# CityU-AIM-Group/SimT

Hardware: AMD Instinct MI355X
Metric: training images/sec at 768x768, DeepLabv2-R101+SimT (higher is better)
Workload: dtype bf16; 1 GPU; DeepLabv2-ResNet101 + SimT(C=19,K=3) full training iteration, batch=4/GPU, 768x768, bf16, 1xMI355X; global_batch=4, inputs=resident in HBM (see h2d_inclusive of a --full run for the PCIe-inclusive rate)

## Files before the change

### simt_amd/csrc/bn_pool.hip

```cpp
#include "common.h"

template <int NJ>
__device__ __forceinline__ void part_colsum8(const float* part, int nblk, int C, int c0, double* out , double (*red)[8][NJ]) {
  const int cl = threadIdx.x & 7, r = threadIdx.x >> 3;
  const int c = c0 + cl;
  double s[NJ];
#pragma unroll
  for (int j = 0; j < NJ; ++j) s[j] = 0.0;
  if (c < C) {
    int b = r;
    for (; b + 96 < nblk; b += 128) {
      float v[4][NJ];
#pragma unroll
      for (int u = 0; u < 4; ++u)
#pragma unroll
        for (int j = 0; j < NJ; ++j) v[u][j] = part[((long)(b + 32 * u) * NJ + j) * C + c];
#pragma unroll
      for (int u = 0; u < 4; ++u)
#pragma unroll
        for (int j = 0; j < NJ; ++j) s[j] += (double)v[u][j];
    }
    for (; b < nblk; b += 32)
#pragma unroll
      for (int j = 0; j < NJ; ++j) s[j] += (double)part[((long)b * NJ + j) * C + c];
// ... 471 lines not shown
    int b = (int)(t / Hp);
    float sc[8], sh[8], best[8];
    int bi[8];
    load8(scale + c, sc);
    load8(shift + c, sh);
#pragma unroll
    for (int e = 0; e < 8; ++e) { best[e] = -INFINITY; bi[e] = 0; }
    bool first = true;
    for (int r = 0; r < 3; ++r) {
      int iy = py * 2 - 1 + r;
      if (iy < 0 || iy >= H) continue;
      for (int s = 0; s < 3; ++s) {
        int ix = px * 2 - 1 + s;
        if (ix < 0 || ix >= W) continue;
        float v[8];
        load8(y + (((long)b * H + iy) * W + ix) * C + c, v);
#pragma unroll
        for (int e = 0; e < 8; ++e) {
          float a = v[e] * sc[e] + sh[e];
          a = a > 0.f ? a : 0.f;
          if (first || a > best[e] || a != a) { best[e] = a; bi[e] = r * 3 + s; }
        }
        first = false;
      }
    }
    store8(p + i * 8, best);
    unsigned long long packed = 0;
#pragma unroll
    for (int e = 0; e < 8; ++e) packed |= (unsigned long long)(bi[e] & 0xff) << (8 * e);
    *(unsigned long long*)(idx + i * 8) = packed;
  }
}

template <typename T>
__global__ void maxpool_bwd_kernel(const T* dp, const unsigned char* idx, T* da, int B, int H, int W, int C, int Hp,
                                   int Wp, long nvec) {
  const int vpr = C >> 3;
  for (long i = (long)blockIdx.x * blockDim.x + threadIdx.x; i < nvec; i += (long)gridDim.x * blockDim.x) {
    int c = (int)(i % vpr) << 3;
    long m = i / vpr;
    int ix = (int)(m % W);
    long t = m / W;
    int iy = (int)(t % H);
    int b = (int)(t / H);
    float acc[8];
#pragma unroll
    for (int e = 0; e < 8; ++e) acc[e] = 0.f;
    int py0 = iy >> 1, px0 = ix >> 1;
    for (int py = py0; py <= ((iy + 1) >> 1); ++py) {
      if (py >= Hp) continue;
      int r = iy - (py * 2 - 1);
      if (r < 0 || r > 2) continue;
      for (int px = px0; px <= ((ix + 1) >> 1); ++px) {
        if (px >= Wp) continue;
        int s = ix - (px * 2 - 1);
        if (s < 0 || s > 2) continue;
        long o = (((long)b * Hp + py) * Wp + px) * C + c;
        unsigned long long packed = *(const unsigned long long*)(idx + o);
        float g[8];
        load8(dp + o, g);
        int want = r * 3 + s;
#pragma unroll
        for (int e = 0; e < 8; ++e)
          if ((int)((packed >> (8 * e)) & 0xff) == want) acc[e] += g[e];
      }
    }
    store8(da + i * 8, acc);
  }
}

extern "C" int simt_bn_relu_maxpool(const void* y, const float* scale, const float* shift, void* p, unsigned char* idx,
                                    int B, int H, int W, int C, int Hp, int Wp, int dtype, simt_stream_t stream) {
  SIMT_CHECK(y && scale && shift && p && idx && C % 8 == 0);
  long nvec = (long)B * Hp * Wp * (C / 8);
  if (dtype == SIMT_BF16)
    hipLaunchKernelGGL(bn_relu_maxpool_kernel<bf16_t>, dim3(ew_grid(nvec)), dim3(256), 0, (hipStream_t)stream,
                       (const bf16_t*)y, scale, shift, (bf16_t*)p, idx, B, H, W, C, Hp, Wp, nvec);
  else
    hipLaunchKernelGGL(bn_relu_maxpool_kernel<float>, dim3(ew_grid(nvec)), dim3(256), 0, (hipStream_t)stream,
                       (const float*)y, scale, shift, (float*)p, idx, B, H, W, C, Hp, Wp, nvec);
  SIMT_LAUNCH_CHECK();
  return SIMT_OK;
}

extern "C" int simt_maxpool_bwd(const void* dp, const unsigned char* idx, void* da, int B, int H, int W, int C, int Hp,
                                int Wp, int dtype, simt_stream_t stream) {
  SIMT_CHECK(dp && idx && da && C % 8 == 0);
  long nvec = (long)B * H * W * (C / 8);
  if (dtype == SIMT_BF16)
    hipLaunchKernelGGL(maxpool_bwd_kernel<bf16_t>, dim3(ew_grid(nvec)), dim3(256), 0, (hipStream_t)stream,
                       (const bf16_t*)dp, idx, (bf16_t*)da, B, H, W, C, Hp, Wp, nvec);
  else
    hipLaunchKernelGGL(maxpool_bwd_kernel<float>, dim3(ew_grid(nvec)), dim3(256), 0, (hipStream_t)stream, (const float*)dp,
                       idx, (float*)da, B, H, W, C, Hp, Wp, nvec);
  SIMT_LAUNCH_CHECK();
  return SIMT_OK;
}

__device__ __forceinline__ long long frag_offset(long long row, long long kcol, int nt16) {
  const long long kt = kcol >> 6, s = (kcol >> 5) & 1, kq = (kcol >> 3) & 3, e = kcol & 7;
  const long long lane = (row & 15) | (kq << 4);
  return ((((kt * nt16 + (row >> 4)) * 2 + s) * 64 + lane) << 3) + e;
}
template <typename T>
__global__ void pack_weight_kernel(const float* w, T* dst, int Cout, int Cin, int RS, int row_off, int tap_off, long ldk,
                                   int Ck, int mode, const float* cscale, long total) {
  for (long i = (long)blockIdx.x * blockDim.x + threadIdx.x; i < total; i += (long)gridDim.x * blockDim.x) {
    int t = (int)(i % RS);
    long r = i / RS;
    int ci = (int)(r % Cin);
    int co = (int)(r / Cin);
    float v = w[i];
    if (cscale) v *= cscale[co];
    const int lm = mode & 0xff, nt16 = mode >> 8;
    const long row = lm == 0 ? (long)(row_off + co) : lm == 1 ? (long)ci : (long)(tap_off + t) * Ck + row_off + co;
    const long kcol = lm == 0 ? (long)(tap_off + t) * Cin + ci : lm == 1 ? (long)(tap_off + t) * Ck + row_off + co : (long)ci;
    const long o = nt16 ? (long)frag_offset(row, kcol, nt16) : row * ldk + kcol;
    Elem<T>::st(dst + o, v);
  }
}

extern "C" int simt_pack_weight(const float* w, void* dst, int Cout, int Cin, int RS, int row_off, int tap_off, long ldk,
                                int Ck, int mode, const float* cscale, int dtype, simt_stream_t stream) {
  SIMT_CHECK(w && dst && Cout > 0 && Cin > 0 && RS > 0);
  long total = (long)Cout * Cin * RS;
  if (dtype == SIMT_BF16)
    hipLaunchKernelGGL(pack_weight_kernel<bf16_t>, dim3(ew_grid(total)), dim3(256), 0, (hipStream_t)stream, w, (bf16_t*)dst,
// ... 312 lines not shown
```

### simt_amd/csrc/common.h

```cpp
#pragma once
#include <hip/hip_runtime.h>
#include <stdint.h>
#include "../../include/simt_hip.h"

typedef unsigned short bf16_t;
typedef __attribute__((ext_vector_type(8))) short bf16x8;
typedef __attribute__((ext_vector_type(4))) short bf16x4;
typedef __attribute__((ext_vector_type(4))) __bf16 bf4v;
typedef __attribute__((ext_vector_type(4))) float f32x4;
typedef __attribute__((ext_vector_type(4))) unsigned int u32x4;

#define GPTR(p) ((const __attribute__((address_space(1))) void*)(p))
#define LPTR(p) ((__attribute__((address_space(3))) void*)(p))

__device__ __forceinline__ float bf2f(bf16_t v) { return __uint_as_float(((uint32_t)v) << 16); }
__device__ __forceinline__ bf16_t f2bf(float f) {
  __bf16 b = (__bf16)f;
  return __builtin_bit_cast(bf16_t, b);
}

__device__ __forceinline__ uint32_t pack_bf16x2(float a, float b) {
  typedef __attribute__((ext_vector_type(2))) float f32x2_t;
  typedef __attribute__((ext_vector_type(2))) __bf16 bf16x2_t;
  const f32x2_t v = {a, b};
// ... 37 lines not shown
}
#ifndef SIMT_NT_STORES
#define SIMT_NT_STORES 0
#endif
static __device__ __forceinline__ void st_out16(void* p, const uint4& v) {
  typedef unsigned simt_u32x4 __attribute__((ext_vector_type(4)));
  const simt_u32x4 w = {v.x, v.y, v.z, v.w};
#if SIMT_NT_STORES
  __builtin_nontemporal_store(w, (simt_u32x4*)p);
#else
  *(simt_u32x4*)p = w;
#endif
}
static __device__ __forceinline__ void st_out8(bf16_t* p, const float* v) {
  uint4 r;
  r.x = pack_bf16x2(v[0], v[1]); r.y = pack_bf16x2(v[2], v[3]); r.z = pack_bf16x2(v[4], v[5]); r.w = pack_bf16x2(v[6], v[7]);
  st_out16(p, r);
}
static __device__ __forceinline__ void st_out8(float* p, const float* v) {
  st_out16(p, make_uint4(__float_as_uint(v[0]), __float_as_uint(v[1]), __float_as_uint(v[2]), __float_as_uint(v[3])));
  st_out16(p + 4, make_uint4(__float_as_uint(v[4]), __float_as_uint(v[5]), __float_as_uint(v[6]), __float_as_uint(v[7])));
}

static __device__ __forceinline__ void store8(float* p, const float* v) { st_out8(p, v); }
static __device__ __forceinline__ void store8(bf16_t* p, const float* v) { st_out8(p, v); }
static __device__ __forceinline__ void st_out16f(float* p, const f32x4& v) {
#if SIMT_NT_STORES
  __builtin_nontemporal_store(v, (f32x4*)p);
#else
  *(f32x4*)p = v;
#endif
}

__device__ __forceinline__ int xcd_remap(int bid, int nwg) {
  int q = nwg >> 3, r = nwg & 7, xcd = bid & 7;
  int base = xcd < r ? xcd * (q + 1) : r * (q + 1) + (xcd - r) * q;
  return base + (bid >> 3);
}

__device__ __forceinline__ float wave_sum(float v) {
#pragma unroll
  for (int o = 32; o > 0; o >>= 1) v += __shfl_xor(v, o, 64);
  return v;
}
__device__ __forceinline__ double wave_sum_d(double v) {
#pragma unroll
  for (int o = 32; o > 0; o >>= 1) v += __shfl_xor(v, o, 64);
  return v;
}

__device__ __forceinline__ void fast_divmod(int m, int d, float rcp, int& q, int& r) {
  q = (int)((float)m * rcp);
  r = m - q * d;
  if (r < 0) { q--; r += d; }
  if (r >= d) { q++; r -= d; }
}

#define SIMT_MAX_DEVICES 16
struct SimtLdsAttrCache { size_t set[SIMT_MAX_DEVICES]; };
static inline bool simt_lds_attr_needed(SimtLdsAttrCache* c, size_t lds) {
  int dev = 0;
  if (hipGetDevice(&dev) != hipSuccess || dev < 0 || dev >= SIMT_MAX_DEVICES) return true;
  if (lds <= c->set[dev]) return false;
  c->set[dev] = lds;
  return true;
}
// ... 20 lines not shown
```

### simt_amd/csrc/head_expand.hip

```cpp
#include "common.h"

struct TapArgs {
  const void* src;
  const float* bias;
  void* dst;
  int B, H, W, Q, QP, lds, ldd, ntaps;
  long M;
  short dy[SIMT_MAX_TAPS], dx[SIMT_MAX_TAPS];
};

__global__ __launch_bounds__(256) void tap_gather_sum_kernel(TapArgs a) {
  const int nq = a.QP >> 2;
  const long total = a.M * nq;
  const float* P = (const float*)a.src;
  float* y = (float*)a.dst;
  for (long idx = (long)blockIdx.x * blockDim.x + threadIdx.x; idx < total; idx += (long)gridDim.x * blockDim.x) {
    const int q = (int)(idx % nq);
    const long m = idx / nq;
    const int ox = (int)(m % a.W);
    const long t2 = m / a.W;
    const int oy = (int)(t2 % a.H);
    float4 acc = make_float4(0.f, 0.f, 0.f, 0.f);
    if (a.bias) {
      const int c = q * 4;
      acc.x = c + 0 < a.Q ? a.bias[c + 0] : 0.f;
      acc.y = c + 1 < a.Q ? a.bias[c + 1] : 0.f;
      acc.z = c + 2 < a.Q ? a.bias[c + 2] : 0.f;
      acc.w = c + 3 < a.Q ? a.bias[c + 3] : 0.f;
    }
    for (int t = 0; t < a.ntaps; ++t) {
      const int iy = oy + a.dy[t], ix = ox + a.dx[t];
      if (iy < 0 || iy >= a.H || ix < 0 || ix >= a.W) continue;
      const float4 v = *(const float4*)(P + (m + (long)a.dy[t] * a.W + a.dx[t]) * a.lds + t * a.QP + q * 4);
      acc.x += v.x; acc.y += v.y; acc.z += v.z; acc.w += v.w;
    }
    *(float4*)(y + m * a.ldd + q * 4) = acc;
  }
}

__global__ __launch_bounds__(256) void tap_scatter_kernel(TapArgs a) {
  const int ng = a.QP >> 3;
  const long total = a.M * a.ntaps * ng;
  const bf16_t* d = (const bf16_t*)a.src;
  bf16_t* G = (bf16_t*)a.dst;
  for (long idx = (long)blockIdx.x * blockDim.x + threadIdx.x; idx < total; idx += (long)gridDim.x * blockDim.x) {
    const int g = (int)(idx % ng);
    long r = idx / ng;
    const int t = (int)(r % a.ntaps);
    const long m = r / a.ntaps;
    const int ox = (int)(m % a.W);
    const int oy = (int)((m / a.W) % a.H);
    const int iy = oy - a.dy[t], ix = ox - a.dx[t];
    uint4 v = make_uint4(0u, 0u, 0u, 0u);
    if (iy >= 0 && iy < a.H && ix >= 0 && ix < a.W)
      v = *(const uint4*)(d + (m - ((long)a.dy[t] * a.W + a.dx[t])) * a.lds + g * 8);
    st_out16(G + m * a.ldd + t * a.QP + g * 8, v);
  }
}

static int tap_grid(long total) {
  long g = (total + 255) / 256;
  if (g > 256 * 16) g = 256 * 16;
  return (int)(g < 1 ? 1 : g);
}

extern "C" int simt_tap_gather_sum(const simt_tap_desc* d, simt_stream_t stream) {
  SIMT_CHECK(d && d->src && d->dst && d->ntaps >= 1 && d->ntaps <= SIMT_MAX_TAPS);
  SIMT_CHECK(d->QP % 4 == 0 && d->lds % 4 == 0 && d->ldd % 4 == 0 && d->QP <= d->ldd && d->ntaps * d->QP <= d->lds);
  TapArgs a;
  a.src = d->src; a.bias = d->bias; a.dst = d->dst; a.B = d->B; a.H = d->H; a.W = d->W; a.Q = d->Q; a.QP = d->QP;
  a.lds = d->lds; a.ldd = d->ldd; a.ntaps = d->ntaps; a.M = (long)d->B * d->H * d->W;
  for (int i = 0; i < SIMT_MAX_TAPS; ++i) { a.dy[i] = d->dy[i]; a.dx[i] = d->dx[i]; }
  hipLaunchKernelGGL(tap_gather_sum_kernel, dim3(tap_grid(a.M * (a.QP / 4))), dim3(256), 0, (hipStream_t)stream, a);
  SIMT_LAUNCH_CHECK();
  return SIMT_OK;
}

extern "C" int simt_tap_scatter(const simt_tap_desc* d, simt_stream_t stream) {
  SIMT_CHECK(d && d->src && d->dst && d->ntaps >= 1 && d->ntaps <= SIMT_MAX_TAPS);
  SIMT_CHECK(d->QP % 8 == 0 && d->lds % 8 == 0 && d->ldd % 8 == 0 && d->QP <= d->lds && d->ntaps * d->QP <= d->ldd);
  TapArgs a;
  a.src = d->src; a.bias = nullptr; a.dst = d->dst; a.B = d->B; a.H = d->H; a.W = d->W; a.Q = d->Q; a.QP = d->QP;
  a.lds = d->lds; a.ldd = d->ldd; a.ntaps = d->ntaps; a.M = (long)d->B * d->H * d->W;
  for (int i = 0; i < SIMT_MAX_TAPS; ++i) { a.dy[i] = d->dy[i]; a.dx[i] = d->dx[i]; }
  hipLaunchKernelGGL(tap_scatter_kernel, dim3(tap_grid(a.M * a.ntaps * (a.QP / 8))), dim3(256), 0, (hipStream_t)stream, a);
  SIMT_LAUNCH_CHECK();
  return SIMT_OK;
}
```

### simt_amd/csrc/head_loss.hip

```cpp
#include "common.h"
#include <math.h>

#define QMAX 40
#ifndef SIMT_HEAD_ABL
#define SIMT_HEAD_ABL 0
#endif
#define NSCAL 13
#define XR_MAX 287

struct HeadGeom {
  int B, h, w, H, W, C, Q, ldp, ldf;
  float sy, sx;
  int half;
  int fix_logits;
  int single;
};

__device__ __forceinline__ float src_coord(int half, float scale, int d) {
  return half ? fmaxf(((float)d + 0.5f) * scale - 0.5f, 0.f) : scale * (float)d;
}
__device__ __forceinline__ void dst_range(int l, int out, float scale, int& lo, int& hi) {
  if (scale > 0.f) {
    const float r = 1.f / scale;
    lo = (int)floorf(((float)l - 1.f) * r) - 2;
    hi = (int)ceilf(((float)l + 2.f) * r) + 2;
  } else { lo = 0; hi = out - 1; }
  lo = max(lo, 0); hi = min(hi, out - 1);
}

struct Taps {
  int o00, o01, o10, o11;
  float wy0, wy1, wx0, wx1;
};

__device__ __forceinline__ Taps make_taps(const HeadGeom& g, int b, int y, int x) {
  Taps t;
  float fy = src_coord(g.half, g.sy, y), fx = src_coord(g.half, g.sx, x);
  int iy0 = (int)fy, ix0 = (int)fx;
  if (iy0 > g.h - 1) iy0 = g.h - 1;
  if (ix0 > g.w - 1) ix0 = g.w - 1;
// ... 102 lines not shown
      m2 = fmaxf(m2, v[j]);
      if (j >= C && v[j] > best) { best = v[j]; y = j; }
    }
  float s2 = exp_le0(0.f - m2);
#pragma unroll
  for (int j = 0; j < QM; ++j)
    if (j < Q && j != arg) s2 += exp_le0(v[j] - m2);
  e.yopen = y; e.m2 = m2; e.sum2 = s2; e.lse2 = m2 + logf(s2);
}

__device__ __forceinline__ unsigned int f32_ord(float f) {
  unsigned int u = __float_as_uint(f);
  return (u & 0x80000000u) ? ~u : (u | 0x80000000u);
}
__device__ __forceinline__ float f32_unord(unsigned int o) {
  unsigned int u = (o & 0x80000000u) ? (o & 0x7fffffffu) : ~o;
  return __uint_as_float(u);
}

__global__ void softmax_rows_kernel(const float* in, int ldi, float* out, int ldo, long M, int C) {
  long m = (long)blockIdx.x * blockDim.x + threadIdx.x;
  if (m >= M) return;
  const float* p = in + m * ldi;
  float mx = p[0];
  for (int c = 1; c < C; ++c) mx = fmaxf(mx, p[c]);
  float s = 0.f;
  for (int c = 0; c < C; ++c) s += expf(p[c] - mx);
  float inv = 1.0f / s;
  float* o = out + m * ldo;
  for (int c = 0; c < C; ++c) o[c] = expf(p[c] - mx) * inv;
  for (int c = C; c < ldo; ++c) o[c] = 0.f;
}

extern "C" int simt_softmax_rows(const float* in, int ldi, float* out, int ldo, long M, int C, simt_stream_t stream) {
  SIMT_CHECK(in && out && C <= ldi && C <= ldo);
  hipLaunchKernelGGL(softmax_rows_kernel, dim3((unsigned)((M + 255) / 256)), dim3(256), 0, (hipStream_t)stream, in, ldi,
                     out, ldo, M, C);
  SIMT_LAUNCH_CHECK();
  return SIMT_OK;
}

struct HeadArgs {
  HeadGeom g;
  const float* pred1;
  const float* pred2;
  const float* fixp;
  const long long* label;
  const float* T1;
  const float* T2;
  float th_high, th_low, lambda_seg, lambda_place;
  float* part;
  unsigned long long* keys;
  float* hout;
  float* g1;
  int QP;
  int rows;
  float gscale;
  int mode;
  unsigned char* conf_out;
  unsigned char* label_ws;
};

__device__ __forceinline__ float wave_sum_dpp63(float v) {
  int x = __float_as_int(v);
#define DPP_ADD(ctrl, rmask)                                                                                  \
  x = __float_as_int(__int_as_float(x) + __int_as_float(__builtin_amdgcn_update_dpp(0, x, ctrl, rmask, 0xf, true)))
  DPP_ADD(0xB1, 0xf);
  DPP_ADD(0x4E, 0xf);
  DPP_ADD(0x141, 0xf);
  DPP_ADD(0x140, 0xf);
// ... 215 lines not shown
              long pp = grp * 256 + wave * 64 + (__ffsll((long long)b1) - 1);
              unsigned long long key = ((unsigned long long)f32_ord(m1) << 32) | (unsigned long long)(0xFFFFFFFFu - (unsigned int)pp);
              atomicMax(&sKey[j], key);
            }
          }
          if (__ballot(live && v2[j] >= best2)) {
            const float a2 = live ? v2[j] : -INFINITY;
            float m2 = wave_max_f(a2);
            unsigned long long b2 = __ballot(live && a2 == m2);
            if (lane == 0 && b2) {
              long pp = grp * 256 + wave * 64 + (__ffsll((long long)b2) - 1);
              unsigned long long key = ((unsigned long long)f32_ord(m2) << 32) | (unsigned long long)(0xFFFFFFFFu - (unsigned int)pp);
              atomicMax(&sKey[QMAX + j], key);
            }
          }
        }
    }
  }

#pragma unroll
  for (int i = 0; i < NSCAL; ++i) {
    float s = wave_sum(acc[i]);
    if (lane == 0) sRed[wave * NSCAL + i] = s;
  }
  __syncthreads();
  float* part = a.part + (long)lbid * (NSCAL + 2 * QC);
  if (tid < NSCAL) part[tid] = sRed[tid] + sRed[NSCAL + tid] + sRed[2 * NSCAL + tid] + sRed[3 * NSCAL + tid];
  for (int i = tid; i < 2 * QC; i += 256)
    part[NSCAL + i] = sdT[i] + sdT[2 * QC + i] + sdT[4 * QC + i] + sdT[6 * QC + i];
  if (tid < 2 * QMAX && sKey[tid]) atomicMax(&a.keys[tid], sKey[tid]);
  if (tid < 2 && sEx[tid]) atomicOr(&a.keys[2 * QMAX + tid], sEx[tid]);
}

__global__ __launch_bounds__(256) void head_reduce_kernel(const float* part, int nblk, int stride, int ncols, double* sums) {
  __shared__ double red[32][8];
  const int cl = threadIdx.x & 7, r = threadIdx.x >> 3;
  const int c = blockIdx.x * 8 + cl;
  double s = 0.0;
  if (c < ncols) {
    int b = r;
    for (; b + 96 < nblk; b += 128) {
      float v[4];
#pragma unroll
      for (int u = 0; u < 4; ++u) v[u] = part[(long)(b + 32 * u) * stride + c];
#pragma unroll
      for (int u = 0; u < 4; ++u) s += (double)v[u];
    }
    for (; b < nblk; b += 32) s += (double)part[(long)b * stride + c];
  }
  red[r][cl] = s;
  __syncthreads();
  if (r == 0 && c < ncols) {
    double t = 0.0;
#pragma unroll
    for (int q = 0; q < 32; ++q) t += red[q][cl];
    sums[c] = t;
  }
}

__device__ __forceinline__ double* head_sums(float* hout, int Q, int C) {
  return (double*)(hout + ((16 + 4 * Q * C + 4 * QMAX + 1) & ~1));
}

__global__ __launch_bounds__(256) void head_finalize_kernel(HeadArgs a, int nblk) {
  const HeadGeom g = a.g;
  const int Q = g.Q, C = g.C, QC = Q * C;
  const int tid = threadIdx.x;
  const double* sc = head_sums(a.hout, Q, C);
  float* o = a.hout;
  const double Np = sc[8], Nk1 = sc[9], Nk2 = sc[10], Ny = sc[11];
  if (tid == 0) {
    o[0] = (float)(sc[0] / Np); o[1] = (float)(sc[1] / Np);
    float k1 = (float)(sc[2] / Nk1), k2 = (float)(sc[3] / Nk2), u1 = (float)(sc[4] / Nk1), u2 = (float)(sc[5] / Nk2);
    o[2] = k1 + a.lambda_place * u1; o[3] = k2 + a.lambda_place * u2;
    o[4] = (float)(sc[6] / Ny); o[5] = (float)(sc[7] / Ny);
    o[6] = (float)Np; o[7] = (float)Nk1; o[8] = (float)Nk2; o[9] = (float)Ny;
    o[10] = k1; o[11] = k2; o[12] = u1; o[13] = u2;
    o[14] = o[1] + a.lambda_seg * o[0];
    o[15] = (float)sc[12];
  }
  float* dTy = o + 16 + 2 * QC + 4 * QMAX;
  for (int i = tid; i < 2 * QC; i += 256) dTy[i] = (float)(-sc[NSCAL + i] / Ny);
  float* ex = o + 16 + 2 * QC;
  float* ai = ex + 2 * QMAX;
  const unsigned long long e1 = a.keys[2 * QMAX], e2 = a.keys[2 * QMAX + 1];
  if (tid < 2 * QMAX) {
    int hd = tid / QMAX, j = tid % QMAX;
    ex[tid] = (j < Q && (((hd ? e2 : e1) >> j) & 1ull)) ? 1.f : 0.f;
    unsigned long long key = a.keys[tid];
    int pidx = (j < Q) ? (int)(0xFFFFFFFFu - (unsigned int)(key & 0xFFFFFFFFull)) : 0;
    ai[tid] = __int_as_float(pidx);
  }
  for (int i = tid; i < 2 * QC; i += 256) {
    if (a.mode != 0) { o[16 + i] = 0.f; continue; }
    int hd = i / QC, r = i % QC, j = r / C, c = r % C;
    unsigned long long key = a.keys[hd * QMAX + j];
    long p = (long)(0xFFFFFFFFu - (unsigned int)(key & 0xFFFFFFFFull));
    int x = (int)(p % g.W);
    long t = p / g.W;
    int y = (int)(t % g.H);
    int b = (int)(t / g.H);
    if (b >= g.B) { b = 0; y = 0; x = 0; }
    Taps tp = make_taps(g, b, y, x);
    const float* f = a.fixp;
    const float vc = lerp4(tp, f[(long)tp.o00 * g.ldf + c], f[(long)tp.o01 * g.ldf + c], f[(long)tp.o10 * g.ldf + c],
                           f[(long)tp.o11 * g.ldf + c]);
    if (!g.fix_logits) { o[16 + i] = vc; continue; }
    float mx = -INFINITY;
    for (int cc = 0; cc < C; ++cc)
      mx = fmaxf(mx, lerp4(tp, f[(long)tp.o00 * g.ldf + cc], f[(long)tp.o01 * g.ldf + cc], f[(long)tp.o10 * g.ldf + cc],
                           f[(long)tp.o11 * g.ldf + cc]));
    float sum = 0.f;
    for (int cc = 0; cc < C; ++cc)
      sum += expf(lerp4(tp, f[(long)tp.o00 * g.ldf + cc], f[(long)tp.o01 * g.ldf + cc], f[(long)tp.o10 * g.ldf + cc],
                        f[(long)tp.o11 * g.ldf + cc]) - mx);
    o[16 + i] = expf(vc - mx) / sum;
  }
}

template <int NB>
__device__ __forceinline__ float run_sum(const float* G, int GP, const float* sL1, int lo, int hi, int mode, float s) {
  if (SIMT_HEAD_ABL & 16) return s;
  float wv[NB * 4], gv[NB * 4];
#pragma unroll
  for (int u = 0; u < NB * 4; ++u) {
    const int pp = max(min(lo + u, hi - 1), 0);
    const float l1 = sL1[pp];
    const float w = mode == 0 ? l1 : mode == 2 ? (1.f - l1) + l1 : 1.f - l1;
    wv[u] = lo + u < hi ? w : 0.f;
    gv[u] = G[pp * GP];
  }
#pragma unroll
  for (int u = 0; u < NB * 4; ++u)
    if (wv[u] != 0.f) s += wv[u] * gv[u];
  return s;
}

#define P2_NACC 18
template <int QM, int QT, int CT, bool... ONE_>
__global__ __launch_bounds__(256, 2) void head_pass2_kernel(HeadArgs a) {
  constexpr bool ONE = (false || ... || ONE_);
  static_assert(!ONE || QT == 0, "the one-head warm-up flavour takes its channel counts at run time (rows = 1)");
  const HeadGeom g = a.g;
  const int Q = QT ? QT : g.Q, C = CT ? CT : g.C, QC = Q * C, QP = a.QP;
  constexpr int CM = CT ? (CT + 3) / 4 * 4 : QM;
  const int GP = Q + 1;
  extern __shared__ __attribute__((aligned(16))) char smem[];
  float* sT = (float*)smem;
  float* sG = sT + 2 * QC;
  float* sAcc = sG + 2 * 256 * GP;
// ... 216 lines not shown
    const float l1 = fy - (float)i0, l0 = 1.f - l1;
    float wk[3];
#pragma unroll
    for (int k = 0; k < 3; ++k) wk[k] = (i0 == iy_first + k ? l0 : 0.f) + (i1 == iy_first + k ? l1 : 0.f);
#pragma unroll
    for (int i = 0; i < NACC; ++i) {
      const int idx = tid + 256 * i;
      if (idx < 2 * g.w * Q) {
        const float sv = sAcc[idx];
#pragma unroll
        for (int k = 0; k < 3; ++k) gacc[k][i] += wk[k] * sv;
      }
    }
    __syncthreads();
  }
  }
  if (GROUPED && R > 1) {
    const int NG = g.H / R, gy = y0 / R;
#pragma unroll
    for (int i = 0; i < NACC; ++i) {
      const int idx = tid + 256 * i;
      if (idx < 2 * g.w * Q) {
        const int hd = idx / (g.w * Q);
        const int r = idx - hd * g.w * Q;
        const int xl = r / Q, j = r - xl * Q;
#pragma unroll
        for (int k = 0; k < 3; ++k)
          a.g1[(((((long)hd * g.B + b) * NG + gy) * 3 + k) * g.w + xl) * QP + j] = gacc[k][i];
      }
    }
  }
}

template <typename T>
__global__ void head_yreduce_kernel(const float* g1, float* d32_1, float* d32_2, T* dT_1, T* dT_2, HeadGeom g, int QP,
                                    int ldo32, int ldoT, long total, int R) {
  long idx = (long)blockIdx.x * blockDim.x + threadIdx.x;
  if (idx >= total) return;
  int j = (int)(idx % QP);
  long t = idx / QP;
  int xl = (int)(t % g.w); t /= g.w;
  int yl = (int)(t % g.h); t /= g.h;
  int b = (int)(t % g.B);
  int hd = (int)(t / g.B);
  if (g.single && hd == 0) return;
  int lo, hi;
  dst_range(yl, g.H, g.sy, lo, hi);
  float s = 0.f;
  if (R > 1) {
    const int NG = g.H / R;
    if (j < g.Q)
      for (int gy = lo / R; gy <= hi / R; ++gy) {
        const int k = yl - min((int)src_coord(g.half, g.sy, gy * R), g.h - 1);
        if (k >= 0 && k < 3) s += g1[(((((long)hd * g.B + b) * NG + gy) * 3 + k) * g.w + xl) * QP + j];
      }
  } else
  for (int yy = lo; yy <= hi; ++yy) {
    float fy = src_coord(g.half, g.sy, yy);
    int i0 = (int)fy;
    if (i0 > g.h - 1) i0 = g.h - 1;
    int i1 = i0 + (i0 < g.h - 1 ? 1 : 0);
    float l1 = fy - (float)i0, l0 = 1.f - l1;
    float wgt = (i0 == yl ? l0 : 0.f) + (i1 == yl ? l1 : 0.f);
    if (wgt != 0.f) s += wgt * g1[((((long)hd * g.B + b) * g.H + yy) * g.w + xl) * QP + j];
  }
  long m = ((long)b * g.h + yl) * g.w + xl;
  float* d32 = hd ? d32_2 : d32_1;
  T* dT = hd ? dT_2 : dT_1;
  if (d32 && j < ldo32) d32[m * ldo32 + j] = s;
  if (dT && j < ldoT) Elem<T>::st(dT + m * ldoT + j, s);
}

static size_t pass1_lds(int Q, int C) {
  size_t QC = (size_t)Q * C;
  return (2 * QC + 8 * QC) * 4 + 8 + (2 * QMAX + 2) * 8 + 4 * NSCAL * 4 + 16;
}
static size_t pass2_lds(int Q, int C, int w) {
  size_t QC = (size_t)Q * C;
  return (2 * QC + 2 * 256 * (size_t)(Q + 1) + 2 * (size_t)w * Q + 512 + XR_MAX + 1) * 4;
}

static int head_rows_per_block(const simt_head_desc* d, float sy) {
  const bool fixed_counts = d->C == 19 && (d->Q == 22 || d->Q == 25);
  if (!fixed_counts || 2l * d->w * d->Q > 256l * P2_NACC) return 1;
  for (int R = 8; R >= 3; --R)
    if (d->H % R == 0 && (float)(R - 1) * sy <= 0.95f && (long)d->B * d->H / R >= 512) return R;
  return 1;
// ... 9 lines not shown
  a.g.B = d->B; a.g.h = d->h; a.g.w = d->w; a.g.H = d->H; a.g.W = d->W; a.g.C = d->C; a.g.Q = d->Q;
  a.g.ldp = d->ldp; a.g.ldf = d->ldf;
  a.g.half = d->up_half_pixel ? 1 : 0; a.g.fix_logits = d->fix_logits ? 1 : 0; a.g.single = d->single ? 1 : 0;
  if (a.g.half) {
    a.g.sy = (float)d->h / (float)d->H;
    a.g.sx = (float)d->w / (float)d->W;
  } else {
    a.g.sy = d->H > 1 ? (float)(d->h - 1) / (float)(d->H - 1) : 0.f;
    a.g.sx = d->W > 1 ? (float)(d->w - 1) / (float)(d->W - 1) : 0.f;
  }
  a.pred1 = d->single ? d->pred2 : d->pred1; a.pred2 = d->pred2; a.fixp = d->fixp; a.label = (const long long*)d->label;
  a.T1 = d->single ? d->T2 : d->T1; a.T2 = d->T2;
  a.th_high = d->th_high; a.th_low = d->th_low; a.lambda_seg = d->lambda_seg; a.lambda_place = d->lambda_place;
  a.part = d->part; a.keys = (unsigned long long*)d->keys; a.hout = d->hout; a.g1 = d->g1; a.QP = d->QP;
  a.gscale = d->gscale;
  a.rows = (d->single && d->mode == 1) ? 1 : head_rows_per_block(d, a.g.sy);
  a.mode = d->mode;
  a.conf_out = d->conf_out;
  a.label_ws = d->label_ws;
  SIMT_CHECK(d->mode == 0 || d->mode == 1);
  return SIMT_OK;
}

extern "C" int simt_head_nblk(int B, int H, int W) {
  long P = (long)B * H * W;
  long n = (P + 255) / 256;
  if (n > 512) n = 512;
  return (int)n;
}
extern "C" int simt_head_part_floats(int Q, int C) { return NSCAL + 2 * Q * C; }
extern "C" int simt_head_hout_floats(int Q, int C) {
  return ((16 + 4 * Q * C + 4 * QMAX + 1) & ~1) + 2 * (NSCAL + 2 * Q * C);
}
extern "C" int simt_head_keys_count(void) { return 2 * QMAX + 2; }

extern "C" int simt_head_loss(const simt_head_desc* d, simt_stream_t stream) {
  HeadArgs a;
  int rc = fill_args(d, a);
  if (rc) return rc;
  hipStream_t st = (hipStream_t)stream;
  const int nblk = simt_head_nblk(d->B, d->H, d->W);
  (void)hipMemsetAsync(d->keys, 0, (2 * QMAX + 2) * sizeof(unsigned long long), st);
  size_t lds1 = pass1_lds(d->Q, d->C);
  SIMT_CHECK(lds1 <= 160 * 1024);
  static SimtLdsAttrCache lds1_cache;
  if (simt_lds_attr_needed(&lds1_cache, lds1)) {
#define P1ATTR(...) (void)hipFuncSetAttribute((const void*)head_pass1_kernel<__VA_ARGS__>, hipFuncAttributeMaxDynamicSharedMemorySize, (int)lds1)
    P1ATTR(24, 22, 19); P1ATTR(28, 25, 19); P1ATTR(24, 0, 0); P1ATTR(QMAX, 0, 0); P1ATTR(24, 0, 0, true); P1ATTR(QMAX, 0, 0, true);
#undef P1ATTR
  }
#define P1(...) hipLaunchKernelGGL((head_pass1_kernel<__VA_ARGS__>), dim3(nblk), dim3(256), lds1, st, a)
  const bool one = d->single && d->mode == 1;
  if (one && d->Q <= 24) P1(24, 0, 0, true);
  else if (one) P1(QMAX, 0, 0, true);
  else if (d->Q == 22 && d->C == 19) P1(24, 22, 19);
  else if (d->Q == 25 && d->C == 19) P1(28, 25, 19);
  else if (d->Q <= 24) P1(24, 0, 0);
  else P1(QMAX, 0, 0);
#undef P1
  SIMT_LAUNCH_CHECK();
  {
    const int ncols = NSCAL + 2 * d->Q * d->C;
    double* sums = (double*)(d->hout + ((16 + 4 * d->Q * d->C + 4 * QMAX + 1) & ~1));
    hipLaunchKernelGGL(head_reduce_kernel, dim3((ncols + 7) / 8), dim3(256), 0, st, d->part, nblk, ncols, ncols, sums);
    SIMT_LAUNCH_CHECK();
  }
  hipLaunchKernelGGL(head_finalize_kernel, dim3(1), dim3(256), 0, st, a, nblk);
  SIMT_LAUNCH_CHECK();
  return SIMT_OK;
}

extern "C" int simt_head_grad(const simt_head_desc* d, simt_stream_t stream) {
  HeadArgs a;
  int rc = fill_args(d, a);
  if (rc) return rc;
  SIMT_CHECK(d->g1 && d->QP >= d->Q);
  hipStream_t st = (hipStream_t)stream;
  size_t lds2 = pass2_lds(d->Q, d->C, d->w);
  SIMT_CHECK(lds2 <= 160 * 1024);
  static SimtLdsAttrCache lds2_cache;
  if (simt_lds_attr_needed(&lds2_cache, lds2)) {
#define P2ATTR(...) (void)hipFuncSetAttribute((const void*)head_pass2_kernel<__VA_ARGS__>, hipFuncAttributeMaxDynamicSharedMemorySize, (int)lds2)
    P2ATTR(24, 22, 19); P2ATTR(28, 25, 19); P2ATTR(24, 0, 0); P2ATTR(QMAX, 0, 0); P2ATTR(24, 0, 0, true); P2ATTR(QMAX, 0, 0, true);
#undef P2ATTR
  }
#define P2(...) hipLaunchKernelGGL((head_pass2_kernel<__VA_ARGS__>), dim3(d->B * d->H / a.rows), dim3(256), lds2, st, a)
  const bool one = d->single && d->mode == 1;
  if (one && d->Q <= 24) P2(24, 0, 0, true);
  else if (one) P2(QMAX, 0, 0, true);
  else if (d->Q == 22 && d->C == 19) P2(24, 22, 19);
  else if (d->Q == 25 && d->C == 19) P2(28, 25, 19);
  else if (d->Q <= 24) P2(24, 0, 0);
  else P2(QMAX, 0, 0);
#undef P2
  SIMT_LAUNCH_CHECK();
  long total = 2l * d->B * d->h * d->w * d->QP;
  unsigned grid = (unsigned)((total + 255) / 256);
  if (d->grad_dtype == SIMT_BF16)
    hipLaunchKernelGGL(head_yreduce_kernel<bf16_t>, dim3(grid), dim3(256), 0, st, d->g1, d->dpred1_f32, d->dpred2_f32,
                       (bf16_t*)d->dpred1_t, (bf16_t*)d->dpred2_t, a.g, d->QP, d->ld_f32, d->ld_t, total, a.rows);
  else
    hipLaunchKernelGGL(head_yreduce_kernel<float>, dim3(grid), dim3(256), 0, st, d->g1, d->dpred1_f32, d->dpred2_f32,
                       (float*)d->dpred1_t, (float*)d->dpred2_t, a.g, d->QP, d->ld_f32, d->ld_t, total, a.rows);
  SIMT_LAUNCH_CHECK();
  return SIMT_OK;
}
```

Baseline: 173.2 images/s.

## Cheapen index math, batch tap loads, fuse head reduce/finalize, vectorize softmax

Adds 32-bit index division when element counts fit, applied to the maxpool backward, tap gather/scatter and yreduce kernels. The 18-tap gather is fully unrolled so all loads are issued before accumulating, and it gains an XCD block remap. The yreduce row loop is batched six at a time. A specialised float4 softmax is added for C≤24. The separate head finalize kernel is folded into the reduce kernel through a last-block atomic ticket, which removes one launch but adds fences and a ticket slot in keys.

```diff
diff --git a/simt_amd/csrc/bn_pool.hip b/simt_amd/csrc/bn_pool.hip
--- a/simt_amd/csrc/bn_pool.hip
+++ b/simt_amd/csrc/bn_pool.hip
@@ -527,17 +527,17 @@
   }
 }
 
-template <typename T>
+template <typename T, bool N32>
 __global__ void maxpool_bwd_kernel(const T* dp, const unsigned char* idx, T* da, int B, int H, int W, int C, int Hp,
                                    int Wp, long nvec) {
   const int vpr = C >> 3;
   for (long i = (long)blockIdx.x * blockDim.x + threadIdx.x; i < nvec; i += (long)gridDim.x * blockDim.x) {
-    int c = (int)(i % vpr) << 3;
-    long m = i / vpr;
-    int ix = (int)(m % W);
-    long t = m / W;
-    int iy = (int)(t % H);
-    int b = (int)(t / H);
+    long m = idx_div<N32>(i, vpr);
+    int c = (int)(i - m * vpr) << 3;
+    long t = idx_div<N32>(m, W);
+    int ix = (int)(m - t * W);
+    int b = (int)idx_div<N32>(t, H);
+    int iy = (int)(t - (long)b * H);
     float acc[8];
 #pragma unroll
     for (int e = 0; e < 8; ++e) acc[e] = 0.f;
@@ -582,12 +582,12 @@
                                 int Wp, int dtype, simt_stream_t stream) {
   SIMT_CHECK(dp && idx && da && C % 8 == 0);
   long nvec = (long)B * H * W * (C / 8);
-  if (dtype == SIMT_BF16)
-    hipLaunchKernelGGL(maxpool_bwd_kernel<bf16_t>, dim3(ew_grid(nvec)), dim3(256), 0, (hipStream_t)stream,
-                       (const bf16_t*)dp, idx, (bf16_t*)da, B, H, W, C, Hp, Wp, nvec);
-  else
-    hipLaunchKernelGGL(maxpool_bwd_kernel<float>, dim3(ew_grid(nvec)), dim3(256), 0, (hipStream_t)stream, (const float*)dp,
-                       idx, (float*)da, B, H, W, C, Hp, Wp, nvec);
+#define POOLB(TT, N32) hipLaunchKernelGGL((maxpool_bwd_kernel<TT, N32>), dim3(ew_grid(nvec)), dim3(256), 0, (hipStream_t)stream, \
+                                          (const TT*)dp, idx, (TT*)da, B, H, W, C, Hp, Wp, nvec)
+  const bool n32 = nvec < (1l << 30);
+  if (dtype == SIMT_BF16) { if (n32) POOLB(bf16_t, true); else POOLB(bf16_t, false); }
+  else { if (n32) POOLB(float, true); else POOLB(float, false); }
+#undef POOLB
   SIMT_LAUNCH_CHECK();
   return SIMT_OK;
 }
diff --git a/simt_amd/csrc/common.h b/simt_amd/csrc/common.h
--- a/simt_amd/csrc/common.h
+++ b/simt_amd/csrc/common.h
@@ -93,6 +93,12 @@
 #endif
 }
 
+template <bool N32>
+__device__ __forceinline__ long idx_div(long x, int d) {
+  if (N32) return (long)((unsigned)x / (unsigned)d);
+  return x / d;
+}
+
 __device__ __forceinline__ int xcd_remap(int bid, int nwg) {
   int q = nwg >> 3, r = nwg & 7, xcd = bid & 7;
   int base = xcd < r ? xcd * (q + 1) : r * (q + 1) + (xcd - r) * q;
diff --git a/simt_amd/csrc/head_expand.hip b/simt_amd/csrc/head_expand.hip
--- a/simt_amd/csrc/head_expand.hip
+++ b/simt_amd/csrc/head_expand.hip
@@ -9,17 +9,21 @@
   short dy[SIMT_MAX_TAPS], dx[SIMT_MAX_TAPS];
 };
 
+#ifndef SIMT_TAP_BATCH
+#define SIMT_TAP_BATCH 1
+#endif
+template <int NT, bool N32>
 __global__ __launch_bounds__(256) void tap_gather_sum_kernel(TapArgs a) {
   const int nq = a.QP >> 2;
   const long total = a.M * nq;
   const float* P = (const float*)a.src;
   float* y = (float*)a.dst;
-  for (long idx = (long)blockIdx.x * blockDim.x + threadIdx.x; idx < total; idx += (long)gridDim.x * blockDim.x) {
-    const int q = (int)(idx % nq);
-    const long m = idx / nq;
-    const int ox = (int)(m % a.W);
-    const long t2 = m / a.W;
-    const int oy = (int)(t2 % a.H);
+  for (long idx = (long)xcd_remap(blockIdx.x, gridDim.x) * blockDim.x + threadIdx.x; idx < total; idx += (long)gridDim.x * blockDim.x) {
+    const long m = idx_div<N32>(idx, nq);
+    const int q = (int)(idx - m * nq);
+    const long t2 = idx_div<N32>(m, a.W);
+    const int ox = (int)(m - t2 * a.W);
+    const int oy = (int)(t2 - idx_div<N32>(t2, a.H) * a.H);
     float4 acc = make_float4(0.f, 0.f, 0.f, 0.f);
     if (a.bias) {
       const int c = q * 4;
@@ -28,28 +32,49 @@
       acc.z = c + 2 < a.Q ? a.bias[c + 2] : 0.f;
       acc.w = c + 3 < a.Q ? a.bias[c + 3] : 0.f;
     }
-    for (int t = 0; t < a.ntaps; ++t) {
-      const int iy = oy + a.dy[t], ix = ox + a.dx[t];
-      if (iy < 0 || iy >= a.H || ix < 0 || ix >= a.W) continue;
-      const float4 v = *(const float4*)(P + (m + (long)a.dy[t] * a.W + a.dx[t]) * a.lds + t * a.QP + q * 4);
-      acc.x += v.x; acc.y += v.y; acc.z += v.z; acc.w += v.w;
+    if constexpr (NT > 0) {
+      float4 v[NT];
+      bool in[NT];
+#pragma unroll
+      for (int t = 0; t < NT; ++t) {
+        const int iy = oy + a.dy[t], ix = ox + a.dx[t];
+        in[t] = iy >= 0 && iy < a.H && ix >= 0 && ix < a.W;
+        const long ms = in[t] ? m + (long)a.dy[t] * a.W + a.dx[t] : m;
+        v[t] = *(const float4*)(P + ms * a.lds + t * a.QP + q * 4);
+      }
+#pragma unroll
+      for (int t = 0; t < NT; ++t) {
+        acc.x = in[t] ? acc.x + v[t].x : acc.x;
+        acc.y = in[t] ? acc.y + v[t].y : acc.y;
+        acc.z = in[t] ? acc.z + v[t].z : acc.z;
+        acc.w = in[t] ? acc.w + v[t].w : acc.w;
+      }
+    } else {
+      for (int t = 0; t < a.ntaps; ++t) {
+        const int iy = oy + a.dy[t], ix = ox + a.dx[t];
+        if (iy < 0 || iy >= a.H || ix < 0 || ix >= a.W) continue;
+        const float4 v = *(const float4*)(P + (m + (long)a.dy[t] * a.W + a.dx[t]) * a.lds + t * a.QP + q * 4);
+        acc.x += v.x; acc.y += v.y; acc.z += v.z; acc.w += v.w;
+      }
     }
     *(float4*)(y + m * a.ldd + q * 4) = acc;
   }
 }
 
+template <bool N32>
 __global__ __launch_bounds__(256) void tap_scatter_kernel(TapArgs a) {
   const int ng = a.QP >> 3;
   const long total = a.M * a.ntaps * ng;
   const bf16_t* d = (const bf16_t*)a.src;
   bf16_t* G = (bf16_t*)a.dst;
   for (long idx = (long)blockIdx.x * blockDim.x + threadIdx.x; idx < total; idx += (long)gridDim.x * blockDim.x) {
-    const int g = (int)(idx % ng);
-    long r = idx / ng;
-    const int t = (int)(r % a.ntaps);
-    const long m = r / a.ntaps;
-    const int ox = (int)(m % a.W);
-    const int oy = (int)((m / a.W) % a.H);
+    const long r = idx_div<N32>(idx, ng);
+    const int g = (int)(idx - r * ng);
+    const long m = idx_div<N32>(r, a.ntaps);
+    const int t = (int)(r - m * a.ntaps);
+    const long t2 = idx_div<N32>(m, a.W);
+    const int ox = (int)(m - t2 * a.W);
+    const int oy = (int)(t2 - idx_div<N32>(t2, a.H) * a.H);
     const int iy = oy - a.dy[t], ix = ox - a.dx[t];
     uint4 v = make_uint4(0u, 0u, 0u, 0u);
     if (iy >= 0 && iy < a.H && ix >= 0 && ix < a.W)
@@ -71,7 +96,15 @@
   a.src = d->src; a.bias = d->bias; a.dst = d->dst; a.B = d->B; a.H = d->H; a.W = d->W; a.Q = d->Q; a.QP = d->QP;
   a.lds = d->lds; a.ldd = d->ldd; a.ntaps = d->ntaps; a.M = (long)d->B * d->H * d->W;
   for (int i = 0; i < SIMT_MAX_TAPS; ++i) { a.dy[i] = d->dy[i]; a.dx[i] = d->dx[i]; }
-  hipLaunchKernelGGL(tap_gather_sum_kernel, dim3(tap_grid(a.M * (a.QP / 4))), dim3(256), 0, (hipStream_t)stream, a);
+  const dim3 grid(tap_grid(a.M * (a.QP / 4)));
+  const bool n32 = a.M * (a.QP / 4) < (1l << 30);
+#define TAP_GATHER(NT, N32) hipLaunchKernelGGL((tap_gather_sum_kernel<NT, N32>), grid, dim3(256), 0, (hipStream_t)stream, a)
+  if (SIMT_TAP_BATCH && a.ntaps == 18) {
+    if (n32) TAP_GATHER(18, true); else TAP_GATHER(18, false);
+  } else {
+    if (n32) TAP_GATHER(0, true); else TAP_GATHER(0, false);
+  }
+#undef TAP_GATHER
   SIMT_LAUNCH_CHECK();
   return SIMT_OK;
 }
@@ -83,7 +116,9 @@
   a.src = d->src; a.bias = nullptr; a.dst = d->dst; a.B = d->B; a.H = d->H; a.W = d->W; a.Q = d->Q; a.QP = d->QP;
   a.lds = d->lds; a.ldd = d->ldd; a.ntaps = d->ntaps; a.M = (long)d->B * d->H * d->W;
   for (int i = 0; i < SIMT_MAX_TAPS; ++i) { a.dy[i] = d->dy[i]; a.dx[i] = d->dx[i]; }
-  hipLaunchKernelGGL(tap_scatter_kernel, dim3(tap_grid(a.M * a.ntaps * (a.QP / 8))), dim3(256), 0, (hipStream_t)stream, a);
+  const long total = a.M * a.ntaps * (a.QP / 8);
+  if (total < (1l << 30)) hipLaunchKernelGGL(tap_scatter_kernel<true>, dim3(tap_grid(total)), dim3(256), 0, (hipStream_t)stream, a);
+  else hipLaunchKernelGGL(tap_scatter_kernel<false>, dim3(tap_grid(total)), dim3(256), 0, (hipStream_t)stream, a);
   SIMT_LAUNCH_CHECK();
   return SIMT_OK;
 }
diff --git a/simt_amd/csrc/head_loss.hip b/simt_amd/csrc/head_loss.hip
--- a/simt_amd/csrc/head_loss.hip
+++ b/simt_amd/csrc/head_loss.hip
@@ -6,6 +6,8 @@
 #define SIMT_HEAD_ABL 0
 #endif
 #define NSCAL 13
+#define HEAD_TICKET (2 * QMAX + 2)
+#define HEAD_KEYS (2 * QMAX + 4)
 #define XR_MAX 287
 
 struct HeadGeom {
@@ -174,10 +176,49 @@
   for (int c = C; c < ldo; ++c) o[c] = 0.f;
 }
 
+#define SM_CMAX 24
+__global__ __launch_bounds__(64) void softmax_rows24_kernel(const float* in, int ldi, float* out, int ldo, long M, int C) {
+  long m = (long)blockIdx.x * blockDim.x + threadIdx.x;
+  if (m >= M) return;
+  const float* p = in + m * ldi;
+  float v[SM_CMAX];
+#pragma unroll
+  for (int c4 = 0; c4 < SM_CMAX / 4; ++c4)
+    if (c4 * 4 < C) {
+      const float4 q = *(const float4*)(p + c4 * 4);
+      v[c4 * 4 + 0] = q.x; v[c4 * 4 + 1] = q.y; v[c4 * 4 + 2] = q.z; v[c4 * 4 + 3] = q.w;
+    }
+  float mx = v[0];
+#pragma unroll
+  for (int c = 1; c < SM_CMAX; ++c)
+    if (c < C) mx = fmaxf(mx, v[c]);
+  float s = 0.f;
+#pragma unroll
+  for (int c = 0; c < SM_CMAX; ++c)
+    if (c < C) { v[c] = expf(v[c] - mx); s += v[c]; }
+  float inv = 1.0f / s;
+  float* o = out + m * ldo;
+#pragma unroll
+  for (int c4 = 0; c4 < SM_CMAX / 4; ++c4)
+    if (c4 * 4 < ldo) {
+      float4 q;
+      q.x = c4 * 4 + 0 < C ? v[c4 * 4 + 0] * inv : 0.f;
+      q.y = c4 * 4 + 1 < C ? v[c4 * 4 + 1] * inv : 0.f;
+      q.z = c4 * 4 + 2 < C ? v[c4 * 4 + 2] * inv : 0.f;
+      q.w = c4 * 4 + 3 < C ? v[c4 * 4 + 3] * inv : 0.f;
+      *(float4*)(o + c4 * 4) = q;
+    }
+  for (int c = SM_CMAX; c < ldo; ++c) o[c] = 0.f;
+}
+
 extern "C" int simt_softmax_rows(const float* in, int ldi, float* out, int ldo, long M, int C, simt_stream_t stream) {
   SIMT_CHECK(in && out && C <= ldi && C <= ldo);
-  hipLaunchKernelGGL(softmax_rows_kernel, dim3((unsigned)((M + 255) / 256)), dim3(256), 0, (hipStream_t)stream, in, ldi,
-                     out, ldo, M, C);
+  const bool vec = C >= 1 && C <= SM_CMAX && ldi % 4 == 0 && ldo % 4 == 0 && ldi >= (C + 3) / 4 * 4 &&
+                   ((uintptr_t)in & 15) == 0 && ((uintptr_t)out & 15) == 0;
+  if (vec)
+    hipLaunchKernelGGL(softmax_rows24_kernel, dim3((unsigned)((M + 63) / 64)), dim3(64), 0, (hipStream_t)stream, in, ldi, out, ldo, M, C);
+  else
+    hipLaunchKernelGGL(softmax_rows_kernel, dim3((unsigned)((M + 63) / 64)), dim3(64), 0, (hipStream_t)stream, in, ldi, out, ldo, M, C);
   SIMT_LAUNCH_CHECK();
   return SIMT_OK;
 }
@@ -459,37 +500,11 @@
   if (tid < 2 && sEx[tid]) atomicOr(&a.keys[2 * QMAX + tid], sEx[tid]);
 }
 
-__global__ __launch_bounds__(256) void head_reduce_kernel(const float* part, int nblk, int stride, int ncols, double* sums) {
-  __shared__ double red[32][8];
-  const int cl = threadIdx.x & 7, r = threadIdx.x >> 3;
-  const int c = blockIdx.x * 8 + cl;
-  double s = 0.0;
-  if (c < ncols) {
-    int b = r;
-    for (; b + 96 < nblk; b += 128) {
-      float v[4];
-#pragma unroll
-      for (int u = 0; u < 4; ++u) v[u] = part[(long)(b + 32 * u) * stride + c];
-#pragma unroll
-      for (int u = 0; u < 4; ++u) s += (double)v[u];
-    }
-    for (; b < nblk; b += 32) s += (double)part[(long)b * stride + c];
-  }
-  red[r][cl] = s;
-  __syncthreads();
-  if (r == 0 && c < ncols) {
-    double t = 0.0;
-#pragma unroll
-    for (int q = 0; q < 32; ++q) t += red[q][cl];
-    sums[c] = t;
-  }
-}
-
 __device__ __forceinline__ double* head_sums(float* hout, int Q, int C) {
   return (double*)(hout + ((16 + 4 * Q * C + 4 * QMAX + 1) & ~1));
 }
 
-__global__ __launch_bounds__(256) void head_finalize_kernel(HeadArgs a, int nblk) {
+__device__ __forceinline__ void head_finalize_body(const HeadArgs& a) {
   const HeadGeom g = a.g;
   const int Q = g.Q, C = g.C, QC = Q * C;
   const int tid = threadIdx.x;
@@ -543,6 +558,48 @@
                         f[(long)tp.o11 * g.ldf + cc]) - mx);
     o[16 + i] = expf(vc - mx) / sum;
   }
+}
+
+__global__ __launch_bounds__(256) void head_reduce_kernel(const float* part, int nblk, int stride, int ncols, double* sums, HeadArgs a) {
+  __shared__ double red[32][8];
+  __shared__ unsigned long long ticket;
+  const int cl = threadIdx.x & 7, r = threadIdx.x >> 3;
+  const int c = blockIdx.x * 8 + cl;
+  double s = 0.0;
+  if (c < ncols) {
+    int b = r;
+    for (; b + 96 < nblk; b += 128) {
+      float v[4];
+#pragma unroll
+      for (int u = 0; u < 4; ++u) v[u] = part[(long)(b + 32 * u) * stride + c];
+#pragma unroll
+      for (int u = 0; u < 4; ++u) s += (double)v[u];
+    }
+    for (; b < nblk; b += 32) s += (double)part[(long)b * stride + c];
+  }
+  red[r][cl] = s;
+  __syncthreads();
+  if (r == 0 && c < ncols) {
+    double t = 0.0;
+#pragma unroll
+    for (int q = 0; q < 32; ++q) t += red[q][cl];
+    sums[c] = t;
+  }
+  asm volatile("s_waitcnt vmcnt(0)" ::: "memory");
+  __syncthreads();
+  if (threadIdx.x == 0) {
+    __builtin_amdgcn_fence(__ATOMIC_RELEASE, "agent");
+    asm volatile("s_waitcnt vmcnt(0)" ::: "memory");
+    ticket = __hip_atomic_fetch_add(a.keys + HEAD_TICKET, 1ull, __ATOMIC_RELAXED, __HIP_MEMORY_SCOPE_AGENT);
+  }
+  __syncthreads();
+  if (ticket != (unsigned long long)gridDim.x - 1) return;
+  if (threadIdx.x == 0) {
+    __builtin_amdgcn_fence(__ATOMIC_ACQUIRE, "agent");
+    asm volatile("s_waitcnt vmcnt(0)" ::: "memory");
+  }
+  __syncthreads();
+  head_finalize_body(a);
 }
 
 template <int NB>
@@ -825,17 +882,20 @@
   }
 }
 
-template <typename T>
+#define YR_B 6
+template <typename T, bool N32>
 __global__ void head_yreduce_kernel(const float* g1, float* d32_1, float* d32_2, T* dT_1, T* dT_2, HeadGeom g, int QP,
                                     int ldo32, int ldoT, long total, int R) {
   long idx = (long)blockIdx.x * blockDim.x + threadIdx.x;
   if (idx >= total) return;
-  int j = (int)(idx % QP);
-  long t = idx / QP;
-  int xl = (int)(t % g.w); t /= g.w;
-  int yl = (int)(t % g.h); t /= g.h;
-  int b = (int)(t % g.B);
-  int hd = (int)(t / g.B);
+  long t = idx_div<N32>(idx, QP);
+  int j = (int)(idx - t * QP);
+  long t1 = idx_div<N32>(t, g.w);
+  int xl = (int)(t - t1 * g.w);
+  long t2 = idx_div<N32>(t1, g.h);
+  int yl = (int)(t1 - t2 * g.h);
+  int hd = (int)idx_div<N32>(t2, g.B);
+  int b = (int)(t2 - (long)hd * g.B);
   if (g.single && hd == 0) return;
   int lo, hi;
   dst_range(yl, g.H, g.sy, lo, hi);
@@ -843,9 +903,20 @@
   if (R > 1) {
     const int NG = g.H / R;
     if (j < g.Q)
-      for (int gy = lo / R; gy <= hi / R; ++gy) {
-        const int k = yl - min((int)src_coord(g.half, g.sy, gy * R), g.h - 1);
-        if (k >= 0 && k < 3) s += g1[(((((long)hd * g.B + b) * NG + gy) * 3 + k) * g.w + xl) * QP + j];
+      for (int gy0 = lo / R; gy0 <= hi / R; gy0 += YR_B) {
+        float v[YR_B];
+        bool use[YR_B];
+#pragma unroll
+        for (int u = 0; u < YR_B; ++u) {
+          const int gy = gy0 + u;
+          const int k = yl - min((int)src_coord(g.half, g.sy, gy * R), g.h - 1);
+          use[u] = gy <= hi / R && k >= 0 && k < 3;
+          v[u] = 0.f;
+          if (use[u]) v[u] = g1[(((((long)hd * g.B + b) * NG + gy) * 3 + k) * g.w + xl) * QP + j];
+        }
+#pragma unroll
+        for (int u = 0; u < YR_B; ++u)
+          if (use[u]) s += v[u];
       }
   } else
   for (int yy = lo; yy <= hi; ++yy) {
@@ -921,7 +992,7 @@
 extern "C" int simt_head_hout_floats(int Q, int C) {
   return ((16 + 4 * Q * C + 4 * QMAX + 1) & ~1) + 2 * (NSCAL + 2 * Q * C);
 }
-extern "C" int simt_head_keys_count(void) { return 2 * QMAX + 2; }
+extern "C" int simt_head_keys_count(void) { return HEAD_KEYS; }
 
 extern "C" int simt_head_loss(const simt_head_desc* d, simt_stream_t stream) {
   HeadArgs a;
@@ -929,7 +1000,7 @@
   if (rc) return rc;
   hipStream_t st = (hipStream_t)stream;
   const int nblk = simt_head_nblk(d->B, d->H, d->W);
-  (void)hipMemsetAsync(d->keys, 0, (2 * QMAX + 2) * sizeof(unsigned long long), st);
+  (void)hipMemsetAsync(d->keys, 0, HEAD_KEYS * sizeof(unsigned long long), st);
   size_t lds1 = pass1_lds(d->Q, d->C);
   SIMT_CHECK(lds1 <= 160 * 1024);
   static SimtLdsAttrCache lds1_cache;
@@ -951,11 +1022,9 @@
   {
     const int ncols = NSCAL + 2 * d->Q * d->C;
     double* sums = (double*)(d->hout + ((16 + 4 * d->Q * d->C + 4 * QMAX + 1) & ~1));
-    hipLaunchKernelGGL(head_reduce_kernel, dim3((ncols + 7) / 8), dim3(256), 0, st, d->part, nblk, ncols, ncols, sums);
+    hipLaunchKernelGGL(head_reduce_kernel, dim3((ncols + 7) / 8), dim3(256), 0, st, d->part, nblk, ncols, ncols, sums, a);
     SIMT_LAUNCH_CHECK();
   }
-  hipLaunchKernelGGL(head_finalize_kernel, dim3(1), dim3(256), 0, st, a, nblk);
-  SIMT_LAUNCH_CHECK();
   return SIMT_OK;
 }
 
@@ -985,12 +1054,12 @@
   SIMT_LAUNCH_CHECK();
   long total = 2l * d->B * d->h * d->w * d->QP;
   unsigned grid = (unsigned)((total + 255) / 256);
-  if (d->grad_dtype == SIMT_BF16)
-    hipLaunchKernelGGL(head_yreduce_kernel<bf16_t>, dim3(grid), dim3(256), 0, st, d->g1, d->dpred1_f32, d->dpred2_f32,
-                       (bf16_t*)d->dpred1_t, (bf16_t*)d->dpred2_t, a.g, d->QP, d->ld_f32, d->ld_t, total, a.rows);
-  else
-    hipLaunchKernelGGL(head_yreduce_kernel<float>, dim3(grid), dim3(256), 0, st, d->g1, d->dpred1_f32, d->dpred2_f32,
-                       (float*)d->dpred1_t, (float*)d->dpred2_t, a.g, d->QP, d->ld_f32, d->ld_t, total, a.rows);
+#define YRED(TT, N32) hipLaunchKernelGGL((head_yreduce_kernel<TT, N32>), dim3(grid), dim3(256), 0, st, d->g1, d->dpred1_f32, d->dpred2_f32, \
+                                        (TT*)d->dpred1_t, (TT*)d->dpred2_t, a.g, d->QP, d->ld_f32, d->ld_t, total, a.rows)
+  const bool n32 = total < (1l << 30);
+  if (d->grad_dtype == SIMT_BF16) { if (n32) YRED(bf16_t, true); else YRED(bf16_t, false); }
+  else { if (n32) YRED(float, true); else YRED(float, false); }
+#undef YRED
   SIMT_LAUNCH_CHECK();
   return SIMT_OK;
 }
```

Result: no change. 173.4 images/s, median of 6 (+0.1%).
